# AKGWSB/EzRT

Measured on AMD Instinct MI355X. Metric: Mrays/s at fixed spp (Bunny ~70k tris, 4 bounces), higher is better.
Workload: dtype f32

## Files before the change

ezrt_amd/csrc/hip/ezrt_internal.h:

```cpp
#pragma once
#include <hip/hip_runtime.h>

#include <algorithm>
#include <array>
#include <chrono>
#include <cstdarg>
#include <cstdio>
#include <cstdlib>
#include <cstring>
#include <exception>
#include <map>
#include <new>
#include <string>
#include <system_error>
#include <thread>
#include <type_traits>
#include <vector>

#include "ezrt.h"
#include "ezrt_device.h"
#include "ezrt_records.h"
#include "ezrt_streams.h"

using namespace ezd;
// ... 120 lines not shown
constexpr int MAX_TRACE_EVENTS = 2048;

struct Tuning {
  int megakernel = 0;
  int leaf_threshold = 12;
  int pool_div = 1;
  int pool_min = 8;
  int pool_max = 128;
  int trace_wps_rel = 7;
  int trace_wps = 6;
  int lds_nodes = 1 << 20;
  int scatter = 1;
  int static_pct = 50;
  int refill_min = 24;
  int lazy_dir = 1;
  int refill_min_rel = 40;
  int rel_boxes = 1;
  int steal = 1;
  int wide4 = 1;
  int debug_stages = 0;
  int debug_oom_above = 0;
  int debug_force_pending = 0;
  int shade_wgs = 0;
  int chunk_log2 = 26;
  int launch_events = 0;
  int env_planes = 1;
  int env_rgbe = 1;
  int min_staged = 16;
  int rel_min_records = 4;
  int gen_primary = 1;
// ... 20 lines not shown
  int lo, hi;
};
const TuningName kTuning[] = {{"megakernel", &Tuning::megakernel, 0, 1},
                              {"leaf_threshold", &Tuning::leaf_threshold, 1, 64},
                              {"pool_div", &Tuning::pool_div, 1, 1 << 16},
                              {"pool_max", &Tuning::pool_max, 8, 4096},
                              {"pool_min", &Tuning::pool_min, 8, 4096},
                              {"trace_wps", &Tuning::trace_wps, 1, 8},
                              {"trace_wps_rel", &Tuning::trace_wps_rel, 0, 8},
                              {"lds_nodes", &Tuning::lds_nodes, 0, 1 << 24},
                              {"steal", &Tuning::steal, 0, 1},
                              {"rel_boxes", &Tuning::rel_boxes, 0, 1},
                              {"refill_min", &Tuning::refill_min, 1, 64},
                              {"refill_min_rel", &Tuning::refill_min_rel, 0, 64},
                              {"lazy_dir", &Tuning::lazy_dir, 0, 1},
                              {"static_pct", &Tuning::static_pct, 0, 95},
                              {"scatter", &Tuning::scatter, 0, 8},
                              {"wide4", &Tuning::wide4, 0, 1},
                              {"debug_stages", &Tuning::debug_stages, 0, 2},
                              {"env_rgbe", &Tuning::env_rgbe, 0, 1},
                              {"env_planes", &Tuning::env_planes, 0, 1},
                              {"launch_events", &Tuning::launch_events, 0, 1},
                              {"shade_wgs", &Tuning::shade_wgs, 0, 4096},
                              {"chunk_log2", &Tuning::chunk_log2, 12, 28},
                              {"debug_force_pending", &Tuning::debug_force_pending, 0, 1 << 20},
                              {"debug_oom_above", &Tuning::debug_oom_above, 0, 1 << 30},
                              {"gen_primary", &Tuning::gen_primary, 0, 1},
                              {"gen_whole", &Tuning::gen_whole, 0, 1},
                              {"rel_min_records", &Tuning::rel_min_records, 0, 4096},
                              {"min_staged", &Tuning::min_staged, 0, 4096},
// ... 241 lines not shown
```

ezrt_amd/csrc/hip/ezrt_kernels.h:

```cpp
#pragma once
#include "ezrt_device.h"
#include "ezrt_records.h"
#include "ezrt_path_device.h"

namespace ezd {

struct TraceArgs {
  DevScene sc;
  EzrtRenderParams p;
  const int2* blocks;
  int32_t n_blocks;
  uint32_t frame_first;
  Sample3* samples;
  unsigned long long* counters;
  int32_t* log_tri;
  float* log_t;
  float* log_colour;
  int32_t stack_entries;
};

EZD bool pixel_owned(const EzrtRenderParams& p, int x, int y) {
  if (x < p.x0 || x >= p.x1 || y < p.y0 || y >= p.y1) return false;
  if (p.shard_count <= 1) return true;
  int tw = p.tile_w > 0 ? p.tile_w : 32, th = p.tile_h > 0 ? p.tile_h : 32;
// ... 66 lines not shown
  const uint32_t blk = s >> 8, tid = s & 255u;
  uint32_t bx, by;
  if (POW2) {
    by = blk >> g.sh_bw;
    bx = blk & ((1u << g.sh_bw) - 1u);
  } else {
    by = fastdiv(blk, g.div_bw);
    bx = blk - by * g.div_bw.d;
  }
  const uint32_t wave = tid >> 6, lane = tid & 63u;
  x = (int)(bx * 16u + (wave & 1u) * 8u + (lane & 7u));
  y = (int)(by * 16u + (wave >> 1) * 8u + (lane >> 3));
  frame = g.frame_first + fk;
}
template <bool POW2>
EZD float4 primary_dir_whole(const GenWhole& g, uint32_t qslot) {
  int x, y;
  uint32_t frame, seed;
  slot_to_pixel_whole<POW2>(g, qslot, x, y, frame);
  const f3 dir = camera_dir_scaled<POW2>(g.sw, g.sh, g.rot, (uint32_t)x, (uint32_t)y, frame, seed);
  return make_float4(dir.x, dir.y, dir.z, 1.0f);
}

template <int INTEG, bool FULLCTR, bool PATHLOG>
__global__ __launch_bounds__(BLOCK) void trace_kernel(TraceArgs a) {
  extern __shared__ __attribute__((aligned(16))) int lds_stack[];
  const int tid = threadIdx.x;
  const int blk = blockIdx.x % a.n_blocks;
  const int fk = blockIdx.x / a.n_blocks;
  const uint32_t frame = a.frame_first + (uint32_t)fk;
  const int wave = tid >> 6, lane = tid & 63;
  const int2 org = a.blocks[blk];
  const int x = org.x + (wave & 1) * 8 + (lane & 7);
  const int y = org.y + (wave >> 1) * 8 + (lane >> 3);
  int* stack = lds_stack + tid;
  const DevScene& sc = a.sc;
// ... 351 lines not shown
```

ezrt_amd/csrc/hip/ezrt_launch.hip:

```cpp
#include "ezrt_internal.h"
#include "ezrt_lds_budget.h"
#include "ezrt_query.h"
#include "ezrt_surface.h"
#include "ezrt_kernels.h"
#include "ezrt_wavefront.h"
#include "ezrt_traceq4.h"

#include <cassert>
#include <climits>

namespace {
using ezi::stack_lds_bytes;
using ezi::with_integrator;

int validate_params(const EzrtScene* s, const EzrtRenderParams* p) {
  if (!p) return fail(EZRT_ERR_INVALID, "params is NULL");
  if (p->width <= 0 || p->height <= 0) return fail(EZRT_ERR_INVALID, "width/height must be positive");
  if (p->x0 < 0 || p->y0 < 0 || p->x1 > p->width || p->y1 > p->height || p->x0 > p->x1 || p->y0 > p->y1)
    return fail(EZRT_ERR_INVALID, "pixel rect outside the image");
  if (p->max_bounce < 0 || p->max_bounce > 64) return fail(EZRT_ERR_INVALID, "max_bounce out of range [0,64]");
  if (!ezi::known_integrator(p->integrator)) return fail(EZRT_ERR_INVALID, "unknown integrator");
  if (p->shard_count < 0 || p->shard_index < 0 || (p->shard_count > 0 && p->shard_index >= p->shard_count))
    return fail(EZRT_ERR_INVALID, "bad shard index/count");
  if (p->tile_w < 0 || p->tile_h < 0) return fail(EZRT_ERR_INVALID, "bad tile size");
// ... 134 lines not shown
}
int gen_whole_mode(const EzrtScene* s, const EzrtRenderParams& p) {
  if (!s->tune.gen_whole || prune_mode(s) != 2) return 0;
  if (p.shard_count > 1 || p.x0 != 0 || p.y0 != 0 || p.x1 != p.width || p.y1 != p.height || p.width % 16 != 0 || p.height % 16 != 0) return 0;
  if (p.width < 16 || p.height < 16) return 0;
  const bool pow2 = (p.width & (p.width - 1)) == 0 && (p.height & (p.height - 1)) == 0;
  return pow2 ? 2 : 1;
}
[[maybe_unused]] bool blocks_are_raster(const EzrtScene* s, const EzrtRenderParams& p) {
  const int bw = p.width / 16, bh = p.height / 16;
  if (!s->blocks_valid || (int)s->blocks_host.size() != bw * bh) return false;
  for (int k = 0; k < bw * bh; k++)
    if (s->blocks_host[k].x != (k % bw) * 16 || s->blocks_host[k].y != (k / bw) * 16) return false;
  return true;
}
int debug_stages_gen_mode(const EzrtScene* s, const EzrtRenderParams& p) {
  return s->tune.debug_stages >= 2 ? 0 : gen_whole_mode(s, p);
}
template <bool REL, bool GEN, bool SEMI, bool GS>
void launch_traceq4_p(int prune, bool log, int wps, int whole, dim3 grid, size_t lds, hipStream_t st, const TraceQ4Args& q) {
  const dim3 block(BLOCK);
  constexpr bool HAS_LOG = GEN || !REL;
  if (prune == 2 || GS) {
    if constexpr (REL && GEN) {
      if (whole && !log) {
        if (wps >= 7) {
          if (whole == 2) hipLaunchKernelGGL((traceq4_kernel<7, REL, false, 2, GEN, SEMI, GS, 2>), grid, block, lds, st, q);
          else hipLaunchKernelGGL((traceq4_kernel<7, REL, false, 2, GEN, SEMI, GS, 1>), grid, block, lds, st, q);
        } else {
          if (whole == 2) hipLaunchKernelGGL((traceq4_kernel<6, REL, false, 2, GEN, SEMI, GS, 2>), grid, block, lds, st, q);
          else hipLaunchKernelGGL((traceq4_kernel<6, REL, false, 2, GEN, SEMI, GS, 1>), grid, block, lds, st, q);
        }
        return;
      }
      if (wps >= 7) {
        if (log) hipLaunchKernelGGL((traceq4_kernel<7, REL, true, 2, GEN, SEMI, GS>), grid, block, lds, st, q);
        else hipLaunchKernelGGL((traceq4_kernel<7, REL, false, 2, GEN, SEMI, GS>), grid, block, lds, st, q);
        return;
      }
    }
    if constexpr (HAS_LOG) {
      if (log) {
        hipLaunchKernelGGL((traceq4_kernel<6, REL, true, 2, GEN, SEMI, GS>), grid, block, lds, st, q);
        return;
      }
// ... 12 lines not shown
  const dim3 grid(c.grid_full);
  int prune = prune_mode(s);
  if (prune == 2 && q.q.rays_per_path == 2u && s->tune.prune_mis != 2) prune = s->tune.prune_mis;
  s->n_trace_launches++;
  const bool log = q.q.wave_log != nullptr;
  const bool semi = !REL && !GEN && (s->tune.semi == 2 || (s->tune.semi == 1 && q.q.rays_per_path == 2u));
  const bool gs = !REL && !GEN && !semi && prune == 2 && q.gscat_shift != 0u;
  if (REL) launch_traceq4_p<REL, GEN, false, false>(prune, log, wps, GEN ? whole : 0, grid, c.lds_t, st, q);
  else if (gs) launch_traceq4_p<false, false, false, true>(prune, log, wps, 0, grid, c.lds_t, st, q);
  else if (semi) launch_traceq4_p<false, false, true, false>(prune, log, wps, 0, grid, c.lds_t, st, q);
  else launch_traceq4_p<false, false, false, false>(prune, log, wps, 0, grid, c.lds_t, st, q);
}
constexpr size_t QHEAD_SLOT_WORDS = (size_t)TRACE_HEADS * TRACE_HEAD_STRIDE;
constexpr size_t QHEADS_WORDS = 81 * QHEAD_SLOT_WORDS;

int fill_traceq4_args(const EzrtScene* s, const TraceCfg& c4, const TraceQArgs& t, const float4* rel, const WfArgs* gen, uint32_t* ovf, TraceQ4Args& A) {
  static_assert(sizeof(GenWhole) <= sizeof(TraceQ4Args::GenGeneral), "the whole-frame generator's arguments lie inside the general one's");
  memset(&A.gen, 0, sizeof A.gen);
  A.gen.div_blocks = A.gen.div_sub = make_fastdiv(1u);
  A.gen.scatter = 1u;
  A.gen.scatter_shift = 6u;
  const int whole = (gen && rel && !t.wave_log) ? gen_whole_mode(s, gen->p) : 0;
  if (whole) {
    GenWhole& w = A.gen_whole;
    const uint32_t bw = (uint32_t)gen->p.width / 16u, n_sub = gen->div_sub.d;
    assert(blocks_are_raster(s, gen->p));
    for (int k = 0; k < 12; k++) w.rot[k] = gen->p.camera_rotate[k];
    w.sw = whole == 2 ? 1.0f / (float)gen->p.width : (float)gen->p.width;
    w.sh = whole == 2 ? 1.0f / (float)gen->p.height : (float)gen->p.height;
    w.div_sub = gen->div_sub;
    w.div_bw = make_fastdiv(bw);
    w.sh_sub = (uint32_t)__builtin_ctz(n_sub);
    w.sh_bw = (uint32_t)__builtin_ctz(bw);
    w.scatter = gen->scatter;
    w.scatter_shift = gen->scatter_shift;
    w.frame_first = gen->frame_first;
  } else if (gen) {
    A.gen.p = gen->p;
    A.gen.blocks = gen->blocks;
    A.gen.div_blocks = gen->div_blocks;
    A.gen.div_sub = gen->div_sub;
    A.gen.scatter = gen->scatter;
    A.gen.scatter_shift = gen->scatter_shift;
    A.gen.frame_first = gen->frame_first;
  }
  A.q = t;
  A.q.stack_entries = (int32_t)(c4.lds / (BLOCK * sizeof(int)));
  A.q.lds_nodes = 0;
  A.q.inner_rel = nullptr;
  if (rel && s->tune.refill_min_rel > 0) A.q.refill_min = (uint32_t)s->tune.refill_min_rel;
  A.inner4 = s->inner4.p;
// ... 3 lines not shown
  {
    const double eps = 1.0 / 16777216.0;
    A.prune_cs = __builtin_nextafterf((float)(2.0 * 17.0 * eps), __builtin_inff());
    A.prune_a = s->prune_a;
    A.tri_leaf = (s->tune.tie_lca && s->tri_leaf.p && s->ref_up.p) ? s->tri_leaf.p : nullptr;
    A.ref_up = s->ref_up.p;
    A.stack_cap = stack_cap4(s);
    A.ovf = ovf;
    A.ovf_cap = ovf ? ovf_cap4(s) : 0;
  }
  A.gscat_shift = (!rel && !gen && !t.slot_map && s->tune.bounce_scatter != 0 && t.rays_per_path == 1u) ? 3u : 0u;
  A.handover = (s->tune.handover && t.steal) ? 1u : 0u;
  A.steal_bound = s->tune.steal_bound ? 1u : 0u;
  return whole;
}
void launch_traceq4_cfg(EzrtScene* s, const TraceCfg& c4, const TraceQArgs& t, const float4* rel, hipStream_t st, const WfArgs* gen, uint32_t* ovf) {
  TraceQ4Args A;
  const int whole = fill_traceq4_args(s, c4, t, rel, gen, ovf, A);
  if (rel && gen) launch_traceq4_rel<true, true>(s, c4, A, whole, st);
  else if (rel) launch_traceq4_rel<true, false>(s, c4, A, 0, st);
  else launch_traceq4_rel<false, false>(s, c4, A, 0, st);
}

void launch_redo(EzrtScene* s, const TraceCfg& cfg, const TraceQArgs& t, uint32_t* head, hipStream_t st) {
  TraceQArgs r = t;
  r.steal = 0u;
  r.count_rays = 0u;
  r.slot_map = t.redo_slots;
  r.n_paths = t.redo_count;
  r.rays_per_path = 1u;
  r.head = head;
  r.dbg = nullptr;
  r.wave_log = nullptr;
  r.force_pending = 0u;
// ... 21 lines not shown
void launch_shade_fused_i(const WfArgs& a, bool full, dim3 grid, hipStream_t st) {
  if (full) {
    if (a.bounce == 0) hipLaunchKernelGGL((shade_kernel<INTEG, true, 0>), grid, dim3(SHADE_BLOCK), 0, st, a);
    else if (a.bounce == 1) hipLaunchKernelGGL((shade_kernel<INTEG, true, 1>), grid, dim3(SHADE_BLOCK), 0, st, a);
    else hipLaunchKernelGGL((shade_kernel<INTEG, true, 2>), grid, dim3(SHADE_BLOCK), 0, st, a);
  } else {
    hipLaunchKernelGGL((shade_kernel<INTEG, false, 2>), grid, dim3(SHADE_BLOCK), 0, st, a);
  }
}
template <int INTEG, int STAGE>
void launch_shade_split_ib(const WfArgs& a, dim3 grid, dim3 grid_hit, hipStream_t st) {
  hipLaunchKernelGGL((shade_miss_kernel<INTEG, false, STAGE>), grid, dim3(SHADE_BLOCK), 0, st, a);
  hipLaunchKernelGGL((shade_hit_kernel<INTEG, false, STAGE>), grid_hit, dim3(SHADE_BLOCK), 0, st, a);
}
template <int INTEG>
void launch_shade_i(const WfArgs& a, bool full, dim3 grid, hipStream_t st) {
  if (!full && a.bounce == 0) launch_shade_split_ib<INTEG, 0>(a, grid, grid, st);
  else if (!full && a.bounce == 1) launch_shade_split_ib<INTEG, 1>(a, grid, grid, st);
  else launch_shade_fused_i<INTEG>(a, full, grid, st);
}
void launch_shade(const WfArgs& a, bool full, dim3 grid, hipStream_t st) {
  with_integrator(a.p.integrator, [&](auto I) { launch_shade_i<decltype(I)::value>(a, full, grid, st); });
}

hipError_t ensure_chunk_scratch(EzrtScene* s, Pipe& pp, size_t n_slots, bool mis, hipStream_t st) {
  if (s->tune.debug_oom_above > 0 && n_slots > (size_t)s->tune.debug_oom_above) return hipErrorOutOfMemory;
  const size_t n_rays_max = n_slots * (mis ? 2 : 1);
#define EZ_ENSURE(x)                   \
  do {                                 \
    hipError_t e_ = (x);               \
    if (e_ != hipSuccess) return e_;   \
  } while (0)
  EZ_ENSURE(pp.samples.ensure(n_slots));
  for (int k = 0; k < 2; k++) {
    EZ_ENSURE(pp.rq_o[k].ensure(n_slots));
    EZ_ENSURE(pp.rq_d[k].ensure(n_rays_max));
    for (int j = 0; j < (mis ? 5 : 4); j++) EZ_ENSURE(pp.st[k][j].ensure(n_slots));
// ... 118 lines not shown
  pro.inner4 = nullptr;
  pro.inner4_rel = nullptr;
  pro.n_inner4 = 0;
  pro.sx = p->eye[0];
  pro.sy = p->eye[1];
  pro.sz = p->eye[2];
  if (wide && s->tune.rel_boxes) {
    HIP_TRY(pp.inner4_rel.ensure((size_t)s->n_inner4 * N4_FLOAT4));
    pro.inner4 = s->inner4.p;
    pro.inner4_rel = pp.inner4_rel.p;
    pro.n_inner4 = s->n_inner4;
  }
  const bool gen_primary = wide && s->tune.rel_boxes && s->tune.gen_primary;
  a.all_owned = (p->shard_count <= 1 && p->x0 == 0 && p->y0 == 0 && p->x1 == p->width && p->y1 == p->height && p->width % 16 == 0 &&
                 p->height % 16 == 0 && s->tune.lazy_dir) ? 1u : 0u;
  a.gen_primary = 0u;
  const bool lean1 = n_slots <= ((size_t)1 << LEAN_SLOT_BITS);
  a.lean1 = lean1 ? 1u : 0u;
  if (gen_primary) hipLaunchKernelGGL(chunk_prologue_kernel, dim3((unsigned)(4 * s->num_cus)), dim3(BLOCK), 0, st, a, pro);
  else hipLaunchKernelGGL(raygen_kernel, dim3((unsigned)((n_slots + BLOCK - 1) / BLOCK)), dim3(BLOCK), 0, st, a, pro);
  if (s->tune.debug_stages && wide)
    fprintf(stderr, "[ezrt] traceq4 launches: %d stack rows (binary tree depth %d); primary stage %d workgroups/CU, %zu B LDS, %d records staged; "
            "bounce stages %d workgroups/CU, %zu B LDS, %d records staged\n", s->stack_need4, s->depth, cfg4_rel.blocks_per_cu, cfg4_rel.lds_t,
            cfg4_rel.lds_nodes, cfg4_abs.blocks_per_cu, cfg4_abs.lds_t, cfg4_abs.lds_nodes);
  if (s->tune.debug_stages && wide && gen_primary) {
    static const char* const kGen[] = {"general", "whole frame", "whole frame, power-of-two"};
    fprintf(stderr, "[ezrt] primary generator: %s\n", kGen[debug_stages_gen_mode(s, *p)]);
  }

  const Tuning& tu = s->tune;
  const TraceCfg cfg = trace_cfg(s);
  const int debug_stages = tu.debug_stages;
  const unsigned trace_grid_full = cfg.grid_full;
  unsigned shade_grid = (unsigned)((n_slots + SHADE_BLOCK - 1) / SHADE_BLOCK);
  unsigned shade_grid_max = s->tune.shade_wgs > 0 ? (unsigned)s->tune.shade_wgs : (unsigned)(12 * s->num_cus);
  if (shade_grid_max > 4096u) shade_grid_max = 4096u;
  if (shade_grid_max < 1u) shade_grid_max = 1u;
  if (shade_grid > shade_grid_max) shade_grid = shade_grid_max;

  for (int b = 0; b <= p->max_bounce; b++) {
    const int in = b & 1, out = in ^ 1;
    TraceQArgs t;
// ... 26 lines not shown
      t.wave_log = pp.wave_log.p;
    }
    int e = tu.launch_events ? s->n_trace_events : MAX_TRACE_EVENTS;
    if (e < MAX_TRACE_EVENTS) {
      while (s->n_trace_events_created <= e) {
        const int ne = s->n_trace_events_created;
        if (!s->ev_trace[ne][0]) HIP_TRY(hipEventCreate(&s->ev_trace[ne][0]));
        if (!s->ev_trace[ne][1]) HIP_TRY(hipEventCreate(&s->ev_trace[ne][1]));
        s->n_trace_events_created = ne + 1;
      }
      HIP_TRY(hipEventRecord(s->ev_trace[e][0], st));
    }
    {
      if (wide) {
        const bool rel = b == 0 && tu.rel_boxes;
        launch_traceq4_cfg(s, rel ? cfg4_rel : cfg4_abs, t, rel ? pp.inner4_rel.p : nullptr, st, (rel && gen_primary) ? &a : nullptr, pp.ovf.p);
      }
      else launch_traceq_cfg(s, cfg, t, false, st);
      if (t.steal || wide) launch_redo(s, cfg, t, pp.qheads.p + (size_t)(40 + b) * HEAD_SLOT, st);
    }
    if (e < MAX_TRACE_EVENTS) {
      HIP_TRY(hipEventRecord(s->ev_trace[e][1], st));
      s->n_trace_events++;
    }
    if (plog) {
      PathLogArgs g;
      g.hits = pp.hits2[in].p;
      g.rq_d = queue(in).d;
      const bool compact = p->integrator == EZRT_INTEGRATOR_P5_SOBOL;
      const bool mis1 = mis && b == 1;
      g.st_slot = (compact || mis1) ? state(in).s1 : state(in).s2;
// ... 25 lines not shown
      g.log_colour = plog->colour;
      g.samples = pp.samples.p;
      hipLaunchKernelGGL(pathlog_kernel, dim3((unsigned)((n_slots + BLOCK - 1) / BLOCK)), dim3(BLOCK), 0, st, g);
    }
    a.hits = pp.hits2[in].p;
    a.hits_out = reinterpret_cast<unsigned long long*>(pp.hits2[out].p);
    a.rq_in = queue(in);
    a.rq_out = queue(out);
    a.st_in = state(in);
    a.st_out = state(out);
    a.n_in = pp.qcounts.p + b;
    a.n_out = pp.qcounts.p + b + 1;
    a.bounce = b;
    a.defer_list = pp.defer_list.p;
    a.defer_count = pp.defer_count.p;
    launch_shade(a, full, dim3(shade_grid), st);
    if (debug_stages) {
      uint32_t q[2] = {0, 0};
      unsigned long long c[EZRT_CTR_COUNT];
      HIP_TRY(hipStreamSynchronize(st));
      HIP_TRY(hipMemcpy(q, pp.qcounts.p + b, sizeof q, hipMemcpyDeviceToHost));
      {
        unsigned long long all[CTR_SLOTS * EZRT_CTR_COUNT];
        HIP_TRY(hipMemcpy(all, s->counters.p, sizeof all, hipMemcpyDeviceToHost));
        for (int k = 0; k < EZRT_CTR_COUNT; k++) {
          c[k] = 0;
          for (int j = 0; j < CTR_SLOTS; j++) c[k] += all[j * EZRT_CTR_COUNT + k];
        }
      }
      if (debug_stages >= 2 && t.wave_log) {
        const size_t nw = (size_t)trace_grid_full * (BLOCK / 64);
// ... 678 lines not shown
```

ezrt_amd/csrc/hip/ezrt_traceq4.h:

```cpp
#pragma once
#include "ezrt_records.h"
#include "ezrt_traceq.h"

namespace ezd {

struct TraceQ4Args {
  TraceQArgs q;
  const float4* inner4;
  const float4* inner4_rel;
  uint32_t root4;
  int32_t lds_nodes4;
  float prune_a, prune_cs;
  const int32_t* tri_leaf;
  const int2* ref_up;
  struct GenGeneral {
    EzrtRenderParams p;
    const int2* blocks;
    FastDiv div_blocks, div_sub;
    uint32_t scatter, scatter_shift, frame_first;
  };
  union {
    GenGeneral gen;
    GenWhole gen_whole;
  };
// ... 115 lines not shown
  bool tie = false;
  bool shared = false;
  int32_t tie_tri = -1;
  bool semi = false;
  bool anyhit = false;
  uint32_t ref = REF_NONE;
  uint32_t n_counted = 0;
  unsigned long long* hits64 = reinterpret_cast<unsigned long long*>(a.hits);
  float prune_t = INF, pdelta = 0.0f;
  auto set_delta = [&]() {
    const float sm = REL ? hw_max3(ez_abs(a.origin[0]), ez_abs(a.origin[1]), ez_abs(a.origin[2])) : hw_max3(ez_abs(S.x), ez_abs(S.y), ez_abs(S.z));
    pdelta = (A.prune_a + A.prune_cs * sm) * hw_max3(ez_abs(inv.x), ez_abs(inv.y), ez_abs(inv.z));
    prune_t = (best_t + pdelta) * PRUNE_REL;
  };
  auto to_redo = [&](uint32_t s) {
    if (atomicExch(&a.redo_flag[s], 1u) == 0u) a.redo_slots[atomicAdd(a.redo_count, 1u)] = s;
    atomicMin(&hits64[s], (unsigned long long)(uint32_t)HIT_PENDING);
  };
  constexpr bool RING = PRUNE == 2;
  const int ring_mask = RING ? A.stack_cap - 1 : -1;
  auto finish = [&]() {
    ref = REF_DONE;
    sp = 0;
    sb = 0;
    if (RING) stack[A.stack_cap * BLOCK] = 0;
  };
  auto pop_or_finish = [&]() {
    if (sp > sb) {
      sp--;
      ref = (uint32_t)stack[(sp & ring_mask) * BLOCK];
// ... 101 lines not shown
          idx = pool_next + r;
          served = true;
          pool_next += cnt;
          if (pool_next >= n_rays && pool_end >= n_rays) exhausted = true;
        }
        uint32_t rs = idx;
        if (gscat) {
          const uint32_t g = idx >> GSH;
          rs = (((g & 255u) * (n_rays >> (8u + GSH)) + (g >> 8)) << GSH) | (idx & ((1u << GSH) - 1u));
        }
        if (need && served && idx < n_rays && rs < n_real) {
          if (a.slot_map) rs = a.slot_map[idx];
          nx_slot = rs;
          if (!REL) nx_o = a.const_origin == 1u ? make_float4(a.origin[0], a.origin[1], a.origin[2], 0.0f) : a.rq.o[rs >> (a.const_origin >> 1)];
          if (GEN) {
            if (WHOLE) nx_d = primary_dir_whole<WHOLE == 2>(A.gen_whole, rs);
            else nx_d = primary_dir(A.gen.p, A.gen.blocks, A.gen.div_blocks, A.gen.div_sub, A.gen.scatter, A.gen.scatter_shift, A.gen.frame_first, rs);
            a.rq.d[rs] = nx_d;
          } else {
            nx_d = a.rq.d[rs];
          }
        }
      }
    }
    if (!ballot((ref & nx_slot) != REF_NONE)) {
      if (!exhausted) continue;
      break;
    }
    if (LOG && a.wave_log && exhausted && !t_exhausted) t_exhausted = wall_clock64();

    if (a.steal && exhausted) {
      if (A.handover) {
        const bool idle0 = (ref & nx_slot) == REF_NONE;
// ... 282 lines not shown
```

ezrt_amd/csrc/hip/ezrt_wavefront.h:

```cpp
#pragma once
#include "ezrt_kernels.h"
#include "ezrt_traceq.h"
#include "ezrt_traceq4.h"

namespace ezd {

constexpr uint32_t FLAG_SHADOW_SHOT = 1u;
constexpr uint32_t FLAG_TERMINATE = 2u;
constexpr uint32_t FLAG_PDF_DEAD = 4u;
struct PathState {
  float4* s0;
  float4* s1;
  float4* s2;
  float4* s3;
  float4* s4;
};
template <int INTEG>
constexpr bool compact_state() { return INTEG == EZRT_INTEGRATOR_P5_SOBOL; }
template <int INTEG, int STAGE>
constexpr bool mis_stage1_state() { return integ_mis<INTEG>() && STAGE == 1; }
struct WfArgs {
  DevScene sc;
  EzrtRenderParams p;
  const int2* blocks;
// ... 7 lines not shown
  const int2* hits;
  unsigned long long* hits_out;
  const uint32_t* n_in;
  uint32_t* n_out;
  int32_t bounce;
  const float* sobol_tab;
  float* sobol_out;
  uint32_t n_frames;
  uint4* defer_list;
  uint32_t* defer_count;
  FastDiv div_blocks;
  FastDiv div_sub;
  uint32_t scatter;
  uint32_t scatter_shift;
  uint32_t all_owned;
  uint32_t gen_primary;
  uint32_t lean1;
};
constexpr uint32_t LEAN_SLOT_BITS = 28u;
constexpr uint32_t LEAN_SLOT_MASK = (1u << LEAN_SLOT_BITS) - 1u;
constexpr uint32_t LEAN_EMITS = 1u << 28;
constexpr uint32_t LEAN_LIVE = 1u << 30;

__global__ __launch_bounds__(BLOCK) void raygen_kernel(WfArgs a, ChunkPrologue g) {
  const uint32_t slot = blockIdx.x * BLOCK + threadIdx.x;
  chunk_prologue(g, slot, gridDim.x * BLOCK);
  if (slot >= a.n_slots) return;
  if (slot == 0) *a.n_out = a.n_slots;
  if (blockIdx.x == 0)
    for (uint32_t k = threadIdx.x; k < a.n_frames * 16u; k += BLOCK)
      a.sobol_out[k] = sobol(k & 15u, gray_code(a.frame_first + (k >> 4) + 1u));
  a.rq_out.d[slot] = primary_dir(a.p, a.blocks, a.div_blocks, a.div_sub, a.scatter, a.scatter_shift, a.frame_first, slot);
// ... 61 lines not shown
  total = lds[NW];
  return lds[wave] + lane_rank(m);
}

struct ShadeOut {
  bool emit;
  uint32_t sslot, seed, flags, tri0;
  f3 history, Lo, Le0, f_r, shadowC, rayL, shadowL, P;
  float cosine, pdf;
};

struct ShadeIn {
  float4 rd4, ro4, s0, s1, s2, s3, s4;
  int2 h, sh;
};
template <int INTEG, int PASS, int STAGE>
EZD void shade_load(const WfArgs& a, const uint32_t i, const bool live, ShadeIn& in, const uint4* entry = nullptr) {
  constexpr bool MIS = integ_mis<INTEG>();
  constexpr bool B0 = (STAGE == 0);
  constexpr bool COMPACT = compact_state<INTEG>();
  constexpr bool MIS1 = mis_stage1_state<INTEG, STAGE>();
  const EzrtRenderParams& p = a.p;
  const int b = a.bounce;
  const uint32_t ii = live ? i : 0u;
  const uint32_t rslot = (b == 0 || !MIS) ? ii : (2u * ii + 1u);
  const bool from_entry = PASS == 2 && entry && (int32_t)entry->y != HIT_PENDING && (!MIS || (int32_t)entry->w != HIT_PENDING);
  int2 h = from_entry ? make_int2((int32_t)entry->y, (int32_t)entry->z) : a.hits[rslot];
  float4 rd4;
  if (B0 && a.gen_primary) {
    rd4 = primary_dir(a.p, a.blocks, a.div_blocks, a.div_sub, a.scatter, a.scatter_shift, a.frame_first, rslot);
  } else if (B0 && PASS == 1 && a.all_owned) {
    asm volatile("" : "+v"(h.x), "+v"(h.y));
    rd4 = make_float4(0.0f, 0.0f, 0.0f, 1.0f);
    if (h.x < 0) rd4 = a.rq_in.d[rslot];
  } else {
    rd4 = a.rq_in.d[rslot];
  }
  const bool lean = COMPACT && STAGE == 1 && a.lean1;
  float4 ro4 = make_float4(p.eye[0], p.eye[1], p.eye[2], 0.0f);
  float4 s0 = make_float4(0, 0, 0, 0), s1 = s0, s2 = s0, s3 = s0, s4 = s0;
  int2 sh = make_int2(-1, 0);
  if (!B0) {
    if (PASS != 1) ro4 = a.rq_in.o[ii];
    if (!COMPACT && !MIS1) s3 = a.st_in.s3[ii];
    s0 = a.st_in.s0[ii];
    if (COMPACT && STAGE == 1) {
      if (!lean) {
        const float2 q = reinterpret_cast<const float2*>(a.st_in.s1)[ii];
        s1 = make_float4(q.x, q.y, 0.0f, 0.0f);
      }
    } else {
      s1 = a.st_in.s1[ii];
    }
    if ((!COMPACT || STAGE >= 2) && !MIS1) s2 = a.st_in.s2[ii];
    if (MIS) {
      s4 = a.st_in.s4[ii];
      sh = from_entry ? make_int2((int32_t)entry->w, 0) : a.hits[2u * ii];
    }
  }
#define EZ_PIN4(v) asm volatile("" : "+v"(v.x), "+v"(v.y), "+v"(v.z), "+v"(v.w))
  EZ_PIN4(rd4);
  asm volatile("" : "+v"(h.x), "+v"(h.y));
  if (!B0) {
    if (PASS != 1) EZ_PIN4(ro4);
    EZ_PIN4(s0);
    if (!lean) EZ_PIN4(s1);
    if ((!COMPACT || STAGE >= 2) && !MIS1) EZ_PIN4(s2);
    if (!COMPACT && !MIS1) EZ_PIN4(s3);
    if (MIS) {
      EZ_PIN4(s4);
      asm volatile("" : "+v"(sh.x), "+v"(sh.y));
    }
  }
#undef EZ_PIN4
  if (lean) {
    const uint32_t w = __float_as_uint(rd4.w);
    uint32_t t0 = 0xffffffffu;
    if (w & LEAN_EMITS) t0 = __float_as_uint(PASS == 1 ? reinterpret_cast<const float*>(a.rq_in.o + ii)[3] : ro4.w);
    s1 = make_float4(__uint_as_float(w & LEAN_SLOT_MASK), __uint_as_float(t0), 0.0f, 0.0f);
  }
  in.rd4 = rd4;
  in.ro4 = ro4;
  in.s0 = s0;
  in.s1 = s1;
  in.s2 = s2;
  in.s3 = s3;
  in.s4 = s4;
  in.h = h;
  in.sh = sh;
}

template <int INTEG, bool FULLCTR, int PASS, int STAGE>
EZD bool shade_body(const WfArgs& a, const uint32_t i, bool live, const ShadeIn& in, Counters& ctr, uint32_t& n_samples,
                    ShadeOut& o) {
  constexpr bool P5TRI = (INTEG >= 50);
  constexpr bool MIS = integ_mis<INTEG>();
  const DevScene& sc = a.sc;
  const EzrtRenderParams& p = a.p;
  const int b = a.bounce;
  constexpr bool B0 = (STAGE == 0);
  constexpr bool COMPACT = compact_state<INTEG>();
  uint32_t sslot = 0, seed = 0, flags = 0, tri0 = 0;
  f3 history = mk(1, 1, 1), Lo = mk(0, 0, 0), Le0 = mk(0, 0, 0), f_r = mk(0, 0, 0), shadowC = mk(0, 0, 0);
  float cosine = 0.0f, pdf = 1.0f;
  f3 rayL = mk(0, 0, 0), shadowL = mk(0, 0, 0);
  Hit hit;
  hit.P = mk(0, 0, 0);
  o.emit = false;
  const float4 rd4 = in.rd4, ro4 = in.ro4, s0 = in.s0, s1 = in.s1, s2 = in.s2, s3 = in.s3, s4 = in.s4;
  const int2 h = in.h, sh = in.sh;
  bool done = false;
  if (!live) return false;
  f3 colour = mk(0, 0, 0);
  const f3 rd = mk(rd4.x, rd4.y, rd4.z);
  if (B0) {
    sslot = queue_to_sample(i, a.div_sub, a.scatter, a.scatter_shift);
    if (rd4.w == 0.0f) {
      live = false;
    } else {
      if (PASS != 2) n_samples = n_samples + 1;
      if (PASS == 1 && h.x == HIT_PENDING) return true;
      if (h.x < 0) {
        colour = hdr_color<FULLCTR>(sc, rd, p.env_clamp, ctr);
        done = true;
      } else {
        if (PASS == 1) return true;
        shade_point<P5TRI>(sc, h.x, __int_as_float(h.y), mk(ro4.x, ro4.y, ro4.z), rd, hit);
        Le0 = hit.m.emissive;
        tri0 = (__float_as_uint(Le0.x) | __float_as_uint(Le0.y) | __float_as_uint(Le0.z)) ? (uint32_t)h.x : 0xffffffffu;
        if (INTEG != EZRT_INTEGRATOR_P5_SOBOL) {
          int x0, y0;
          uint32_t f0;
          slot_to_pixel(a.blocks, a.div_blocks, sslot, a.frame_first, x0, y0, f0);
          seed = ((uint32_t)x0 * 1973u + (uint32_t)y0 * 9277u + f0 * 26699u) | 1u;
          wang_hash(seed);
          wang_hash(seed);
        }
      }
    }
  } else {
    if (!MIS && rd4.w == 0.0f) return false;
    if (COMPACT) {
      cosine = s0.w;
      pdf = 1.0f / (2.0f * PI);
      if (STAGE == 1) {
// ... 204 lines not shown
    a.rq_out.d[2u * k + 1u] = make_float4(o.rayL.x, o.rayL.y, o.rayL.z, shoot ? 1.0f : 0.0f);
  } else {
    a.rq_out.o[k] = make_float4(o.P.x, o.P.y, o.P.z, ow);
    a.rq_out.d[k] = make_float4(o.rayL.x, o.rayL.y, o.rayL.z, dw);
  }
}
template <int INTEG, int STAGE>
constexpr int store_form() { return compact_state<INTEG>() ? (STAGE == 0 ? 1 : 2) : ((integ_mis<INTEG>() && STAGE == 0) ? 3 : 0); }
template <bool MIS, int FORM>
EZD void shade_emit(const WfArgs& a, const ShadeOut& o, uint32_t* alloc_lds) {
  const uint32_t k = block_alloc(a.n_out, o.emit, alloc_lds);
  if (!o.emit) return;
  shade_store<MIS, FORM>(a, o, k);
}

template <int INTEG, bool FULLCTR, int STAGE>
__global__ __launch_bounds__(SHADE_BLOCK, SHADE_MISS_WAVES) void shade_miss_kernel(WfArgs a) {
  constexpr bool B0 = (STAGE == 0);
  __shared__ uint32_t list_tail;
  const uint32_t n_in = B0 ? a.n_slots : *a.n_in;
  const uint32_t stride = gridDim.x * SHADE_BLOCK;
  const uint32_t iters = (n_in + stride - 1) / stride;
  uint4* list = a.defer_list + (size_t)blockIdx.x * iters * SHADE_BLOCK;
  if (threadIdx.x == 0) list_tail = 0u;
  __syncthreads();
  Counters ctr = {0, 0, 0, 0, 0, 0, 0};
  uint32_t n_samples = 0;
  const int lane = threadIdx.x & 63;
  for (uint32_t k = 0, i = blockIdx.x * SHADE_BLOCK + threadIdx.x; k < iters; k++, i += stride) {
    ShadeOut o;
    ShadeIn in;
    shade_load<INTEG, 1, STAGE>(a, i, i < n_in, in);
    const bool deferred = shade_body<INTEG, FULLCTR, 1, STAGE>(a, i, i < n_in, in, ctr, n_samples, o);
    const unsigned long long m = ballot(deferred);
    if (m) {
      uint32_t base = 0;
      if (lane == 0) base = atomicAdd(&list_tail, (uint32_t)__popcll(m));
      base = (uint32_t)__builtin_amdgcn_readfirstlane((int)base);
      if (deferred) list[base + lane_rank(m)] = make_uint4(i, (uint32_t)in.h.x, (uint32_t)in.h.y, (uint32_t)in.sh.x);
    }
  }
  __syncthreads();
  if (threadIdx.x == 0) a.defer_count[blockIdx.x] = list_tail;
  if (B0) {
    unsigned long long sn = wave_sum(n_samples);
    if (lane == 0 && sn) atomicAdd(&ctr_slot(a.counters)[EZRT_CTR_SAMPLES], sn);
  }
  if (FULLCTR) {
    unsigned long long v5 = wave_sum(ctr.envmap), v6 = wave_sum(ctr.envcache);
    if (lane == 0) {
      atomicAdd(&ctr_slot(a.counters)[EZRT_CTR_ENV_MAP], v5);
      atomicAdd(&ctr_slot(a.counters)[EZRT_CTR_ENV_CACHE], v6);
    }
  }
}

template <int INTEG, bool FULLCTR, int STAGE>
__global__ __launch_bounds__(SHADE_BLOCK, (integ_mis<INTEG>() && STAGE == 0) ? 6 : 4) void shade_hit_kernel(WfArgs a) {
  __shared__ uint32_t alloc_lds[SHADE_BLOCK / 64 + 1];
  constexpr bool B0 = (STAGE == 0);
  constexpr int FORM = store_form<INTEG, STAGE>();
  constexpr bool MIS = integ_mis<INTEG>();
  const uint32_t n_in = B0 ? a.n_slots : *a.n_in;
  const uint32_t stride = gridDim.x * SHADE_BLOCK;
  const uint32_t iters = (n_in + stride - 1) / stride;
  const uint4* list = a.defer_list + (size_t)blockIdx.x * iters * SHADE_BLOCK;
  const uint32_t cnt = a.defer_count[blockIdx.x];
  auto shade_entry = [&](const uint4 e, Counters& c, uint32_t& ns, ShadeOut& o) {
    ShadeIn in;
    shade_load<INTEG, 2, STAGE>(a, e.x, true, in, &e);
    shade_body<INTEG, FULLCTR, 2, STAGE>(a, e.x, true, in, c, ns, o);
  };
  Counters ctr = {0, 0, 0, 0, 0, 0, 0};
  uint32_t n_samples = 0;
  if (!MIS) {
    if (cnt == 0u) return;
    if (threadIdx.x == 0) alloc_lds[0] = (a.bounce < a.p.max_bounce) ? atomicAdd(a.n_out, cnt) : 0u;
    __syncthreads();
    const uint32_t base = alloc_lds[0];
    for (uint32_t j = threadIdx.x; j < cnt; j += SHADE_BLOCK) {
      ShadeOut o;
      shade_entry(list[j], ctr, n_samples, o);
      if (o.emit) shade_store<MIS, FORM>(a, o, base + j);
      else if (a.bounce < a.p.max_bounce)
        a.rq_out.d[base + j] = make_float4(0.0f, 0.0f, 0.0f, 0.0f);
    }
// ... 208 lines not shown
```

Baseline: 15630.

## Regenerate primary ray directions in shading instead of storing them from trace

For Sobol-based integrators with the whole-frame generator, the primary trace kernel stops writing generated ray directions to the ray queue, except for rays sent to the redo path. The first-bounce shade miss and hit kernels instead recompute each direction (and the camera seed) from the slot index. This removes a float4 global store per primary ray and the matching load in shading, at the cost of redoing the camera-direction arithmetic and adding new template instances.

```diff
diff --git a/ezrt_amd/csrc/hip/ezrt_internal.h b/ezrt_amd/csrc/hip/ezrt_internal.h
--- a/ezrt_amd/csrc/hip/ezrt_internal.h
+++ b/ezrt_amd/csrc/hip/ezrt_internal.h
@@ -158,6 +158,7 @@
   int static_pct = 50;
   int refill_min = 24;
   int lazy_dir = 1;
+  int regen_dir = 1;
   int refill_min_rel = 40;
   int rel_boxes = 1;
   int steal = 1;
@@ -208,6 +209,7 @@
                               {"refill_min", &Tuning::refill_min, 1, 64},
                               {"refill_min_rel", &Tuning::refill_min_rel, 0, 64},
                               {"lazy_dir", &Tuning::lazy_dir, 0, 1},
+                              {"regen_dir", &Tuning::regen_dir, 0, 1},
                               {"static_pct", &Tuning::static_pct, 0, 95},
                               {"scatter", &Tuning::scatter, 0, 8},
                               {"wide4", &Tuning::wide4, 0, 1},
diff --git a/ezrt_amd/csrc/hip/ezrt_kernels.h b/ezrt_amd/csrc/hip/ezrt_kernels.h
--- a/ezrt_amd/csrc/hip/ezrt_kernels.h
+++ b/ezrt_amd/csrc/hip/ezrt_kernels.h
@@ -104,12 +104,17 @@
   frame = g.frame_first + fk;
 }
 template <bool POW2>
-EZD float4 primary_dir_whole(const GenWhole& g, uint32_t qslot) {
+EZD float4 primary_dir_whole(const GenWhole& g, uint32_t qslot, uint32_t& seed) {
   int x, y;
-  uint32_t frame, seed;
+  uint32_t frame;
   slot_to_pixel_whole<POW2>(g, qslot, x, y, frame);
   const f3 dir = camera_dir_scaled<POW2>(g.sw, g.sh, g.rot, (uint32_t)x, (uint32_t)y, frame, seed);
   return make_float4(dir.x, dir.y, dir.z, 1.0f);
+}
+template <bool POW2>
+EZD float4 primary_dir_whole(const GenWhole& g, uint32_t qslot) {
+  uint32_t seed;
+  return primary_dir_whole<POW2>(g, qslot, seed);
 }
 
 template <int INTEG, bool FULLCTR, bool PATHLOG>
diff --git a/ezrt_amd/csrc/hip/ezrt_launch.hip b/ezrt_amd/csrc/hip/ezrt_launch.hip
--- a/ezrt_amd/csrc/hip/ezrt_launch.hip
+++ b/ezrt_amd/csrc/hip/ezrt_launch.hip
@@ -172,6 +172,14 @@
     if (s->blocks_host[k].x != (k % bw) * 16 || s->blocks_host[k].y != (k / bw) * 16) return false;
   return true;
 }
+#ifndef EZRT_REGEN_PARTS
+#define EZRT_REGEN_PARTS 7
+#endif
+int regen_dir_mode(const EzrtScene* s, const EzrtRenderParams& p, bool gen_primary, bool audit) {
+  if (!s->tune.regen_dir || !gen_primary || audit || s->instr > 0 || s->tune.debug_stages >= 2) return 0;
+  if (p.integrator < EZRT_INTEGRATOR_P5_SOBOL || gen_whole_mode(s, p) != 2) return 0;
+  return (EZRT_REGEN_PARTS & 7) == 7 ? 2 : ((EZRT_REGEN_PARTS & 3) ? 1 : 0);
+}
 int debug_stages_gen_mode(const EzrtScene* s, const EzrtRenderParams& p) {
   return s->tune.debug_stages >= 2 ? 0 : gen_whole_mode(s, p);
 }
@@ -183,10 +191,12 @@
     if constexpr (REL && GEN) {
       if (whole && !log) {
         if (wps >= 7) {
-          if (whole == 2) hipLaunchKernelGGL((traceq4_kernel<7, REL, false, 2, GEN, SEMI, GS, 2>), grid, block, lds, st, q);
+          if (whole == 3) hipLaunchKernelGGL((traceq4_kernel<7, REL, false, 2, GEN, SEMI, GS, 3>), grid, block, lds, st, q);
+          else if (whole == 2) hipLaunchKernelGGL((traceq4_kernel<7, REL, false, 2, GEN, SEMI, GS, 2>), grid, block, lds, st, q);
           else hipLaunchKernelGGL((traceq4_kernel<7, REL, false, 2, GEN, SEMI, GS, 1>), grid, block, lds, st, q);
         } else {
-          if (whole == 2) hipLaunchKernelGGL((traceq4_kernel<6, REL, false, 2, GEN, SEMI, GS, 2>), grid, block, lds, st, q);
+          if (whole == 3) hipLaunchKernelGGL((traceq4_kernel<6, REL, false, 2, GEN, SEMI, GS, 3>), grid, block, lds, st, q);
+          else if (whole == 2) hipLaunchKernelGGL((traceq4_kernel<6, REL, false, 2, GEN, SEMI, GS, 2>), grid, block, lds, st, q);
           else hipLaunchKernelGGL((traceq4_kernel<6, REL, false, 2, GEN, SEMI, GS, 1>), grid, block, lds, st, q);
         }
         return;
@@ -229,6 +239,21 @@
 constexpr size_t QHEAD_SLOT_WORDS = (size_t)TRACE_HEADS * TRACE_HEAD_STRIDE;
 constexpr size_t QHEADS_WORDS = 81 * QHEAD_SLOT_WORDS;
 
+void fill_gen_whole(const EzrtScene* s, const WfArgs& gen, int whole, GenWhole& w) {
+  const uint32_t bw = (uint32_t)gen.p.width / 16u, n_sub = gen.div_sub.d;
+  assert(blocks_are_raster(s, gen.p));
+  (void)s;
+  for (int k = 0; k < 12; k++) w.rot[k] = gen.p.camera_rotate[k];
+  w.sw = whole == 2 ? 1.0f / (float)gen.p.width : (float)gen.p.width;
+  w.sh = whole == 2 ? 1.0f / (float)gen.p.height : (float)gen.p.height;
+  w.div_sub = gen.div_sub;
+  w.div_bw = make_fastdiv(bw);
+  w.sh_sub = (uint32_t)__builtin_ctz(n_sub);
+  w.sh_bw = (uint32_t)__builtin_ctz(bw);
+  w.scatter = gen.scatter;
+  w.scatter_shift = gen.scatter_shift;
+  w.frame_first = gen.frame_first;
+}
 int fill_traceq4_args(const EzrtScene* s, const TraceCfg& c4, const TraceQArgs& t, const float4* rel, const WfArgs* gen, uint32_t* ovf, TraceQ4Args& A) {
   static_assert(sizeof(GenWhole) <= sizeof(TraceQ4Args::GenGeneral), "the whole-frame generator's arguments lie inside the general one's");
   memset(&A.gen, 0, sizeof A.gen);
@@ -237,19 +262,7 @@
   A.gen.scatter_shift = 6u;
   const int whole = (gen && rel && !t.wave_log) ? gen_whole_mode(s, gen->p) : 0;
   if (whole) {
-    GenWhole& w = A.gen_whole;
-    const uint32_t bw = (uint32_t)gen->p.width / 16u, n_sub = gen->div_sub.d;
-    assert(blocks_are_raster(s, gen->p));
-    for (int k = 0; k < 12; k++) w.rot[k] = gen->p.camera_rotate[k];
-    w.sw = whole == 2 ? 1.0f / (float)gen->p.width : (float)gen->p.width;
-    w.sh = whole == 2 ? 1.0f / (float)gen->p.height : (float)gen->p.height;
-    w.div_sub = gen->div_sub;
-    w.div_bw = make_fastdiv(bw);
-    w.sh_sub = (uint32_t)__builtin_ctz(n_sub);
-    w.sh_bw = (uint32_t)__builtin_ctz(bw);
-    w.scatter = gen->scatter;
-    w.scatter_shift = gen->scatter_shift;
-    w.frame_first = gen->frame_first;
+    fill_gen_whole(s, *gen, whole, A.gen_whole);
   } else if (gen) {
     A.gen.p = gen->p;
     A.gen.blocks = gen->blocks;
@@ -283,10 +296,12 @@
   A.steal_bound = s->tune.steal_bound ? 1u : 0u;
   return whole;
 }
-void launch_traceq4_cfg(EzrtScene* s, const TraceCfg& c4, const TraceQArgs& t, const float4* rel, hipStream_t st, const WfArgs* gen, uint32_t* ovf) {
+void launch_traceq4_cfg(EzrtScene* s, const TraceCfg& c4, const TraceQArgs& t, const float4* rel, hipStream_t st, const WfArgs* gen, uint32_t* ovf,
+                        bool keep_dirs = true) {
   TraceQ4Args A;
   const int whole = fill_traceq4_args(s, c4, t, rel, gen, ovf, A);
-  if (rel && gen) launch_traceq4_rel<true, true>(s, c4, A, whole, st);
+  assert(keep_dirs || whole == 2);
+  if (rel && gen) launch_traceq4_rel<true, true>(s, c4, A, (whole == 2 && !keep_dirs) ? 3 : whole, st);
   else if (rel) launch_traceq4_rel<true, false>(s, c4, A, 0, st);
   else launch_traceq4_rel<false, false>(s, c4, A, 0, st);
 }
@@ -338,13 +353,25 @@
   hipLaunchKernelGGL((shade_hit_kernel<INTEG, false, STAGE>), grid_hit, dim3(SHADE_BLOCK), 0, st, a);
 }
 template <int INTEG>
-void launch_shade_i(const WfArgs& a, bool full, dim3 grid, hipStream_t st) {
-  if (!full && a.bounce == 0) launch_shade_split_ib<INTEG, 0>(a, grid, grid, st);
+void launch_shade_regen_i(const WfArgs& a, dim3 grid, hipStream_t st) {
+  if constexpr (INTEG >= EZRT_INTEGRATOR_P5_SOBOL) {
+    if (EZRT_REGEN_PARTS & 1) hipLaunchKernelGGL((shade_miss_kernel<INTEG, false, STAGE_REGEN>), grid, dim3(SHADE_BLOCK), 0, st, a);
+    else hipLaunchKernelGGL((shade_miss_kernel<INTEG, false, 0>), grid, dim3(SHADE_BLOCK), 0, st, a);
+    if (EZRT_REGEN_PARTS & 2) hipLaunchKernelGGL((shade_hit_kernel<INTEG, false, STAGE_REGEN>), grid, dim3(SHADE_BLOCK), 0, st, a);
+    else hipLaunchKernelGGL((shade_hit_kernel<INTEG, false, 0>), grid, dim3(SHADE_BLOCK), 0, st, a);
+  } else {
+    launch_shade_split_ib<INTEG, 0>(a, grid, grid, st);
+  }
+}
+template <int INTEG>
+void launch_shade_i(const WfArgs& a, bool full, bool regen, dim3 grid, hipStream_t st) {
+  if (!full && a.bounce == 0 && regen) launch_shade_regen_i<INTEG>(a, grid, st);
+  else if (!full && a.bounce == 0) launch_shade_split_ib<INTEG, 0>(a, grid, grid, st);
   else if (!full && a.bounce == 1) launch_shade_split_ib<INTEG, 1>(a, grid, grid, st);
   else launch_shade_fused_i<INTEG>(a, full, grid, st);
 }
-void launch_shade(const WfArgs& a, bool full, dim3 grid, hipStream_t st) {
-  with_integrator(a.p.integrator, [&](auto I) { launch_shade_i<decltype(I)::value>(a, full, grid, st); });
+void launch_shade(const WfArgs& a, bool full, bool regen, dim3 grid, hipStream_t st) {
+  with_integrator(a.p.integrator, [&](auto I) { launch_shade_i<decltype(I)::value>(a, full, regen, grid, st); });
 }
 
 hipError_t ensure_chunk_scratch(EzrtScene* s, Pipe& pp, size_t n_slots, bool mis, hipStream_t st) {
@@ -493,7 +520,9 @@
   const bool gen_primary = wide && s->tune.rel_boxes && s->tune.gen_primary;
   a.all_owned = (p->shard_count <= 1 && p->x0 == 0 && p->y0 == 0 && p->x1 == p->width && p->y1 == p->height && p->width % 16 == 0 &&
                  p->height % 16 == 0 && s->tune.lazy_dir) ? 1u : 0u;
-  a.gen_primary = 0u;
+  const int regen = regen_dir_mode(s, *p, gen_primary, plog != nullptr);
+  memset(&a.gen_whole, 0, sizeof a.gen_whole);
+  if (regen) fill_gen_whole(s, a, 2, a.gen_whole);
   const bool lean1 = n_slots <= ((size_t)1 << LEAN_SLOT_BITS);
   a.lean1 = lean1 ? 1u : 0u;
   if (gen_primary) hipLaunchKernelGGL(chunk_prologue_kernel, dim3((unsigned)(4 * s->num_cus)), dim3(BLOCK), 0, st, a, pro);
@@ -505,6 +534,7 @@
   if (s->tune.debug_stages && wide && gen_primary) {
     static const char* const kGen[] = {"general", "whole frame", "whole frame, power-of-two"};
     fprintf(stderr, "[ezrt] primary generator: %s\n", kGen[debug_stages_gen_mode(s, *p)]);
+    fprintf(stderr, "[ezrt] primary directions: %s\n", regen ? "regenerated" : "stored");
   }
 
   const Tuning& tu = s->tune;
@@ -561,7 +591,8 @@
     {
       if (wide) {
         const bool rel = b == 0 && tu.rel_boxes;
-        launch_traceq4_cfg(s, rel ? cfg4_rel : cfg4_abs, t, rel ? pp.inner4_rel.p : nullptr, st, (rel && gen_primary) ? &a : nullptr, pp.ovf.p);
+        launch_traceq4_cfg(s, rel ? cfg4_rel : cfg4_abs, t, rel ? pp.inner4_rel.p : nullptr, st, (rel && gen_primary) ? &a : nullptr, pp.ovf.p,
+                           !(rel && regen == 2));
       }
       else launch_traceq_cfg(s, cfg, t, false, st);
       if (t.steal || wide) launch_redo(s, cfg, t, pp.qheads.p + (size_t)(40 + b) * HEAD_SLOT, st);
@@ -617,7 +648,7 @@
     a.bounce = b;
     a.defer_list = pp.defer_list.p;
     a.defer_count = pp.defer_count.p;
-    launch_shade(a, full, dim3(shade_grid), st);
+    launch_shade(a, full, b == 0 && regen > 0, dim3(shade_grid), st);
     if (debug_stages) {
       uint32_t q[2] = {0, 0};
       unsigned long long c[EZRT_CTR_COUNT];
diff --git a/ezrt_amd/csrc/hip/ezrt_traceq4.h b/ezrt_amd/csrc/hip/ezrt_traceq4.h
--- a/ezrt_amd/csrc/hip/ezrt_traceq4.h
+++ b/ezrt_amd/csrc/hip/ezrt_traceq4.h
@@ -153,6 +153,7 @@
     prune_t = (best_t + pdelta) * PRUNE_REL;
   };
   auto to_redo = [&](uint32_t s) {
+    if constexpr (GEN && WHOLE == 3) a.rq.d[s] = make_float4(d.x, d.y, d.z, 1.0f);
     if (atomicExch(&a.redo_flag[s], 1u) == 0u) a.redo_slots[atomicAdd(a.redo_count, 1u)] = s;
     atomicMin(&hits64[s], (unsigned long long)(uint32_t)HIT_PENDING);
   };
@@ -284,9 +285,9 @@
           nx_slot = rs;
           if (!REL) nx_o = a.const_origin == 1u ? make_float4(a.origin[0], a.origin[1], a.origin[2], 0.0f) : a.rq.o[rs >> (a.const_origin >> 1)];
           if (GEN) {
-            if (WHOLE) nx_d = primary_dir_whole<WHOLE == 2>(A.gen_whole, rs);
+            if (WHOLE) nx_d = primary_dir_whole<WHOLE >= 2>(A.gen_whole, rs);
             else nx_d = primary_dir(A.gen.p, A.gen.blocks, A.gen.div_blocks, A.gen.div_sub, A.gen.scatter, A.gen.scatter_shift, A.gen.frame_first, rs);
-            a.rq.d[rs] = nx_d;
+            if (WHOLE != 3) a.rq.d[rs] = nx_d;
           } else {
             nx_d = a.rq.d[rs];
           }
diff --git a/ezrt_amd/csrc/hip/ezrt_wavefront.h b/ezrt_amd/csrc/hip/ezrt_wavefront.h
--- a/ezrt_amd/csrc/hip/ezrt_wavefront.h
+++ b/ezrt_amd/csrc/hip/ezrt_wavefront.h
@@ -45,8 +45,8 @@
   uint32_t scatter;
   uint32_t scatter_shift;
   uint32_t all_owned;
-  uint32_t gen_primary;
   uint32_t lean1;
+  GenWhole gen_whole;
 };
 constexpr uint32_t LEAN_SLOT_BITS = 28u;
 constexpr uint32_t LEAN_SLOT_MASK = (1u << LEAN_SLOT_BITS) - 1u;
@@ -138,7 +138,7 @@
   float4 rd4, ro4, s0, s1, s2, s3, s4;
   int2 h, sh;
 };
-template <int INTEG, int PASS, int STAGE>
+template <int INTEG, int PASS, int STAGE, bool REGEN = false>
 EZD void shade_load(const WfArgs& a, const uint32_t i, const bool live, ShadeIn& in, const uint4* entry = nullptr) {
   constexpr bool MIS = integ_mis<INTEG>();
   constexpr bool B0 = (STAGE == 0);
@@ -151,8 +151,9 @@
   const bool from_entry = PASS == 2 && entry && (int32_t)entry->y != HIT_PENDING && (!MIS || (int32_t)entry->w != HIT_PENDING);
   int2 h = from_entry ? make_int2((int32_t)entry->y, (int32_t)entry->z) : a.hits[rslot];
   float4 rd4;
-  if (B0 && a.gen_primary) {
-    rd4 = primary_dir(a.p, a.blocks, a.div_blocks, a.div_sub, a.scatter, a.scatter_shift, a.frame_first, rslot);
+  static_assert(!REGEN || (B0 && PASS != 0), "the regenerating instances are the primary stage's two passes");
+  if constexpr (REGEN) {
+    rd4 = make_float4(0.0f, 0.0f, 0.0f, 1.0f);
   } else if (B0 && PASS == 1 && a.all_owned) {
     asm volatile("" : "+v"(h.x), "+v"(h.y));
     rd4 = make_float4(0.0f, 0.0f, 0.0f, 1.0f);
@@ -182,8 +183,13 @@
       sh = from_entry ? make_int2((int32_t)entry->w, 0) : a.hits[2u * ii];
     }
   }
+  if constexpr (REGEN && PASS == 2) {
+    uint32_t seed;
+    rd4 = primary_dir_whole<true>(a.gen_whole, rslot, seed);
+    s3.w = __uint_as_float(seed);
+  }
 #define EZ_PIN4(v) asm volatile("" : "+v"(v.x), "+v"(v.y), "+v"(v.z), "+v"(v.w))
-  EZ_PIN4(rd4);
+  if constexpr (!REGEN) EZ_PIN4(rd4);
   asm volatile("" : "+v"(h.x), "+v"(h.y));
   if (!B0) {
     if (PASS != 1) EZ_PIN4(ro4);
@@ -214,7 +220,7 @@
   in.sh = sh;
 }
 
-template <int INTEG, bool FULLCTR, int PASS, int STAGE>
+template <int INTEG, bool FULLCTR, int PASS, int STAGE, bool REGEN = false>
 EZD bool shade_body(const WfArgs& a, const uint32_t i, bool live, const ShadeIn& in, Counters& ctr, uint32_t& n_samples,
                     ShadeOut& o) {
   constexpr bool P5TRI = (INTEG >= 50);
@@ -236,7 +242,7 @@
   bool done = false;
   if (!live) return false;
   f3 colour = mk(0, 0, 0);
-  const f3 rd = mk(rd4.x, rd4.y, rd4.z);
+  f3 rd = mk(rd4.x, rd4.y, rd4.z);
   if (B0) {
     sslot = queue_to_sample(i, a.div_sub, a.scatter, a.scatter_shift);
     if (rd4.w == 0.0f) {
@@ -245,6 +251,10 @@
       if (PASS != 2) n_samples = n_samples + 1;
       if (PASS == 1 && h.x == HIT_PENDING) return true;
       if (h.x < 0) {
+        if constexpr (REGEN && PASS == 1) {
+          const float4 g = primary_dir_whole<true>(a.gen_whole, i);
+          rd = mk(g.x, g.y, g.z);
+        }
         colour = hdr_color<FULLCTR>(sc, rd, p.env_clamp, ctr);
         done = true;
       } else {
@@ -252,7 +262,9 @@
         shade_point<P5TRI>(sc, h.x, __int_as_float(h.y), mk(ro4.x, ro4.y, ro4.z), rd, hit);
         Le0 = hit.m.emissive;
         tri0 = (__float_as_uint(Le0.x) | __float_as_uint(Le0.y) | __float_as_uint(Le0.z)) ? (uint32_t)h.x : 0xffffffffu;
-        if (INTEG != EZRT_INTEGRATOR_P5_SOBOL) {
+        if constexpr (REGEN) {
+          seed = __float_as_uint(s3.w);
+        } else if (INTEG != EZRT_INTEGRATOR_P5_SOBOL) {
           int x0, y0;
           uint32_t f0;
           slot_to_pixel(a.blocks, a.div_blocks, sslot, a.frame_first, x0, y0, f0);
@@ -487,8 +499,11 @@
   shade_store<MIS, FORM>(a, o, k);
 }
 
-template <int INTEG, bool FULLCTR, int STAGE>
+constexpr int STAGE_REGEN = 3;
+template <int INTEG, bool FULLCTR, int STAGE_>
 __global__ __launch_bounds__(SHADE_BLOCK, SHADE_MISS_WAVES) void shade_miss_kernel(WfArgs a) {
+  constexpr bool REGEN = (STAGE_ == STAGE_REGEN);
+  constexpr int STAGE = REGEN ? 0 : STAGE_;
   constexpr bool B0 = (STAGE == 0);
   __shared__ uint32_t list_tail;
   const uint32_t n_in = B0 ? a.n_slots : *a.n_in;
@@ -503,8 +518,8 @@
   for (uint32_t k = 0, i = blockIdx.x * SHADE_BLOCK + threadIdx.x; k < iters; k++, i += stride) {
     ShadeOut o;
     ShadeIn in;
-    shade_load<INTEG, 1, STAGE>(a, i, i < n_in, in);
-    const bool deferred = shade_body<INTEG, FULLCTR, 1, STAGE>(a, i, i < n_in, in, ctr, n_samples, o);
+    shade_load<INTEG, 1, STAGE, REGEN>(a, i, i < n_in, in);
+    const bool deferred = shade_body<INTEG, FULLCTR, 1, STAGE, REGEN>(a, i, i < n_in, in, ctr, n_samples, o);
     const unsigned long long m = ballot(deferred);
     if (m) {
       uint32_t base = 0;
@@ -528,9 +543,11 @@
   }
 }
 
-template <int INTEG, bool FULLCTR, int STAGE>
-__global__ __launch_bounds__(SHADE_BLOCK, (integ_mis<INTEG>() && STAGE == 0) ? 6 : 4) void shade_hit_kernel(WfArgs a) {
+template <int INTEG, bool FULLCTR, int STAGE_>
+__global__ __launch_bounds__(SHADE_BLOCK, (integ_mis<INTEG>() && (STAGE_ == 0 || STAGE_ == STAGE_REGEN)) ? 6 : 4) void shade_hit_kernel(WfArgs a) {
   __shared__ uint32_t alloc_lds[SHADE_BLOCK / 64 + 1];
+  constexpr bool REGEN = (STAGE_ == STAGE_REGEN);
+  constexpr int STAGE = REGEN ? 0 : STAGE_;
   constexpr bool B0 = (STAGE == 0);
   constexpr int FORM = store_form<INTEG, STAGE>();
   constexpr bool MIS = integ_mis<INTEG>();
@@ -541,8 +558,8 @@
   const uint32_t cnt = a.defer_count[blockIdx.x];
   auto shade_entry = [&](const uint4 e, Counters& c, uint32_t& ns, ShadeOut& o) {
     ShadeIn in;
-    shade_load<INTEG, 2, STAGE>(a, e.x, true, in, &e);
-    shade_body<INTEG, FULLCTR, 2, STAGE>(a, e.x, true, in, c, ns, o);
+    shade_load<INTEG, 2, STAGE, REGEN>(a, e.x, true, in, &e);
+    shade_body<INTEG, FULLCTR, 2, STAGE, REGEN>(a, e.x, true, in, c, ns, o);
   };
   Counters ctr = {0, 0, 0, 0, 0, 0, 0};
   uint32_t n_samples = 0;
```

Result: faster. 15860, median of 6 (+1.5%).
